# Zhongxu-Wang/ArtSpeech

Hardware: AMD Instinct MI355X
Metric: mel frames/sec (whole job; per-GPU = value / n_gpus), acoustic-model inference path, batch 32 x 200-frame utterances (higher is better)
Workload: dtype f32 (f16x3 split-operand MFMA, fp32 accumulate)

## Files before the change

artspeech_amd/csrc/conv_gemm.h:

```cpp
#pragma once
#include "artspeech_hip.h"
#include "common.h"
#include "conv_gemm_rule.h"
#include "operand_image.h"

#define OOB 0xFFFFFFFFu
#define OOBH 0x80000000u

int as_conv_gemm_h3_launch(const ConvGemmArgs* const* a, const int* S, int n, int choice, hipStream_t stream);
int as_split_f16x2_launch(const float* x, int ldx, int K, int N, int lrelu, float slope, uint16_t* xh, hipStream_t stream,
                          const int32_t* n_valid = nullptr);

static inline __host__ __device__ int as_kbx(int K) { return operand_image::kbx(K); }
static inline bool as_fills_tall_tile(int M) { return conv_gemm_rule::fills_tall_tile(M); }

static inline conv_gemm_rule::Shape as_conv_gemm_shape(const ConvGemmArgs& a)
{
    conv_gemm_rule::Shape s;
    s.M = a.M; s.N = a.N; s.K = a.K; s.Kp = a.Kp; s.T = a.T; s.K2 = a.K2;
    s.n_prod = a.n_prod ? a.n_prod : 3;
    s.n_groups = a.n_groups < 1 ? 1 : a.n_groups;
    s.group_cols = a.group_cols; s.ileave_u = a.ileave_u; s.act = a.act;
    s.x32 = a.X != nullptr; s.xh = a.Xh != nullptr; s.y32 = a.Y != nullptr; s.yh = a.Yh != nullptr; s.w32 = a.W != nullptr;
    s.res = a.res != nullptr; s.div_sqrt2 = a.div_sqrt2 != 0; s.transpose_out = a.transpose_out != 0;
    s.has_ws = a.ws != nullptr; s.ws_bytes = a.ws_bytes;
    return s;
}
size_t as_conv_gemm_shape_workspace(const conv_gemm_rule::Shape& s, bool set);

struct H3Taps {
    unsigned long long w0, w1, w2, w3;
    int wide;
};

static inline int h3_pack_taps(const ConvGemmArgs& a, H3Taps* out)
{
    H3Taps tp = {0, 0, 0, 0, 0};
    unsigned long long* w = &tp.w0;
    for (int t = 0; t < a.T; ++t)
        if (a.dh[t] < -7 || a.dh[t] > 7 || a.dw[t] < -7 || a.dw[t] > 7) tp.wide = 1;
    for (int t = 0; t < a.T; ++t) {
        if (tp.wide && (a.dh[t] != 0 || a.dw[t] < -127 || a.dw[t] > 127)) return AS_EINVAL;
        const int byte = tp.wide ? a.dw[t] + 128 : ((a.dh[t] + 8) << 4) | (a.dw[t] + 8);
        w[t >> 3] |= (unsigned long long)byte << ((t & 7) * 8);
    }
    *out = tp;
    return AS_OK;
}

#ifdef __HIPCC__
static __device__ __forceinline__ unsigned long long h3_tap_word(const H3Taps& tp, int t)
{
    const int s = t >> 3;
    const unsigned long long m0 = 0ull - (unsigned long long)(s == 0), m1 = 0ull - (unsigned long long)(s == 1),
                             m2 = 0ull - (unsigned long long)(s == 2), m3 = 0ull - (unsigned long long)(s == 3);
    return (tp.w0 & m0) | (tp.w1 & m1) | (tp.w2 & m2) | (tp.w3 & m3);
}

#endif

#ifdef __HIPCC__
typedef float f32x16 __attribute__((ext_vector_type(16)));
typedef float f32x4 __attribute__((ext_vector_type(4)));
typedef unsigned u32x2_t __attribute__((ext_vector_type(2)));
typedef _Float16 f16x8 __attribute__((ext_vector_type(8)));

static __device__ __forceinline__ f32x4 buf_load4(__amdgpu_buffer_rsrc_t r, unsigned voff, int soff)
{
    return __builtin_bit_cast(f32x4, __builtin_amdgcn_raw_buffer_load_b128(r, voff, soff, 0));
}
static __device__ __forceinline__ float buf_load1(__amdgpu_buffer_rsrc_t r, unsigned voff, int soff)
{
    return __builtin_bit_cast(float, __builtin_amdgcn_raw_buffer_load_b32(r, voff, soff, 0));
}
#define H3_MAXP 6
struct H3Prob {
    ConvGemmArgs a;
    H3Taps tp;
    int32_t wg0, wgs;
    int32_t tiles, S;
    int32_t col0, col1;
    int32_t pad0_, pad1_;
};
struct H3Multi {
    int32_t n, pad_;
    H3Prob p[H3_MAXP];
};

static __device__ __forceinline__ int logical_of(int local, int wgs)
{
    return (local & 7) * (wgs >> 3) + (local >> 3);
}

static __device__ __forceinline__ float div_sqrt2f(float x)
{
    const float c = 1.41421356237309504880f, rc = 0.70710678118654752440f;
    const float q = x * rc;
    return __builtin_fmaf(__builtin_fmaf(-q, c, x), rc, q);
}

template <int ACT>
static __device__ __forceinline__ float epi_act(float x, float slope)
{
    if (ACT == 1) x = x < 0.f ? 0.f : x;
    if (ACT == 2) x = x > 0.f ? x : slope * x;
    if (ACT == 3) x = tanhf(x);
    if (ACT == 4) x = fabsf(x);
    if (ACT == 5) x = x / (1.0f + expf(-x));
    return x;
}

static __device__ __forceinline__ void yh_store_tile(const ConvGemmArgs& a, __amdgpu_buffer_rsrc_t rsH, const float (&v)[16], int row0,
                                                     int col, int lk, int n_end)
{
    const unsigned NXy = operand_image::rows32(a.N);
    const int groups = 2 * as_kbx(a.M);
#pragma unroll
    for (int pr = 0; pr < 2; ++pr) {
        float t[8];
#pragma unroll
        for (int r = 0; r < 4; ++r) {
            float x0 = v[8 * pr + r], x1 = v[8 * pr + 4 + r];
            if (a.yh_lrelu) {
                x0 = x0 > 0.f ? x0 : a.in_slope * x0;
                x1 = x1 > 0.f ? x1 : a.in_slope * x1;
            }
            asm volatile("s_nop 1\n\tv_permlane32_swap_b32 %0, %1" : "+v"(x0), "+v"(x1));
            t[r] = x0;
            t[4 + r] = x1;
        }
        u32x4_t h, l;
        split2(t, h, l);
        const int g = (row0 >> 3) + 2 * pr + lk;
        const bool ok = col < n_end && g < groups;
        const unsigned off = ok ? operand_image::byte_off(operand_image::plane(g), col, NXy) : OOBH;
        __builtin_amdgcn_raw_buffer_store_b128(h, rsH, off, 0, 0);
        __builtin_amdgcn_raw_buffer_store_b128(l, rsH, off + 2u * NXy * 16u, 0, 0);
        if (col == 0 && g < groups) {
            const u32x4_t z = {0u, 0u, 0u, 0u};
            const unsigned offz = operand_image::byte_off(operand_image::plane(g), a.N, NXy);
            __builtin_amdgcn_raw_buffer_store_b128(z, rsH, offz, 0, 0);
            __builtin_amdgcn_raw_buffer_store_b128(z, rsH, offz + 2u * NXy * 16u, 0, 0);
        }
    }
}

template <int TM, int TN, bool DIV, int ACT, bool TR>
static __device__ __forceinline__ void epilogue_tiles(const ConvGemmArgs& a, const f32x16 (&acc)[TM][TN], int rbase, int cbase,
                                                      int l31, int lk, int grp, int n_end)
{
    const __amdgpu_buffer_rsrc_t rsB = __builtin_amdgcn_make_buffer_rsrc(
        const_cast<float*>(a.bias ? a.bias + (size_t)grp * a.M : nullptr), 0, a.bias ? a.M * 4 : 0, 0x00020000);
    const __amdgpu_buffer_rsrc_t rsR = __builtin_amdgcn_make_buffer_rsrc(
        const_cast<float*>(a.res), 0, a.res ? (int)((unsigned)a.M * a.ldr * 4u) : 0, 0x00020000);
    const __amdgpu_buffer_rsrc_t rsY = __builtin_amdgcn_make_buffer_rsrc(
        a.Y, 0, a.Y ? (int)((unsigned)(TR ? a.N : (a.ileave_u > 1 ? a.M / a.ileave_u : a.M)) * a.ldy * 4u) : 0, 0x00020000);
    const __amdgpu_buffer_rsrc_t rsH = __builtin_amdgcn_make_buffer_rsrc(
        a.Yh, 0, a.Yh ? (int)operand_image::desc_bytes(a.M, operand_image::rows32(a.N)) : 0, 0x00020000);
    const float sc = a.acc_scale;
    if (a.range_probe) {
        bool bad = false;
#pragma unroll
        for (int i = 0; i < TM; ++i)
#pragma unroll
            for (int jn = 0; jn < TN; ++jn)
#pragma unroll
                for (int e = 0; e < 16; ++e) bad |= !(fabsf(acc[i][jn][e]) <= 3.0e38f);
        if (bad) as_status_raise(a.status, AS_STATUS_F16_RANGE);
    }
    float bv[TM][16];
#pragma unroll
    for (int i = 0; i < TM; ++i)
#pragma unroll
        for (int e = 0; e < 16; ++e) bv[i][e] = 0.f;
    if (a.bias) {
#pragma unroll
        for (int i = 0; i < TM; ++i)
#pragma unroll
            for (int e = 0; e < 16; ++e)
                bv[i][e] = buf_load1(rsB, (unsigned)(rbase + i * 32 + (e & 3) + 8 * (e >> 2)) * 4u, 0);
    }
#pragma unroll
    for (int i = 0; i < TM; ++i) {
#pragma unroll
        for (int jn = 0; jn < TN; ++jn) {
            const int col = cbase + jn * 32 + l31;
            const int row0 = rbase + i * 32;
            const unsigned r_off = col < n_end ? (unsigned)(row0 * a.ldr + col) * 4u : OOBH;
            float v[16];
#pragma unroll
            for (int e = 0; e < 16; ++e) v[e] = 0.f;
            if (a.res) {
#pragma unroll
                for (int e = 0; e < 16; ++e) v[e] = buf_load1(rsR, r_off + (unsigned)(((e & 3) + 8 * (e >> 2)) * a.ldr * 4), 0);
            }
#pragma unroll
            for (int e = 0; e < 16; ++e) {
                float x = __builtin_fmaf(acc[i][jn][e], sc, bv[i][e]);
                x += v[e];
                if (DIV) x = div_sqrt2f(x);
                v[e] = epi_act<ACT>(x, a.act_slope);
            }
            if (TR) {
                const bool quad = (a.ldy & 3) == 0 && (reinterpret_cast<uintptr_t>(a.Y) & 15) == 0 && row0 + 28 <= a.M;
                const unsigned off = col < n_end ? (unsigned)(col * a.ldy + row0) * 4u : OOBH;
                if (quad) {
#pragma unroll
                    for (int q = 0; q < 4; ++q) {
                        const f32x4 t = {v[4 * q], v[4 * q + 1], v[4 * q + 2], v[4 * q + 3]};
                        __builtin_amdgcn_raw_buffer_store_b128(__builtin_bit_cast(u32x4_t, t), rsY, off + 32u * q, 0, 0);
                    }
                } else {
#pragma unroll
                    for (int e = 0; e < 16; ++e) {
                        const int dr = (e & 3) + 8 * (e >> 2);
                        __builtin_amdgcn_raw_buffer_store_b32(__builtin_bit_cast(unsigned, v[e]), rsY,
                                                              row0 + dr < a.M ? off + 4u * dr : OOBH, 0, 0);
                    }
                }
            } else {
                if (a.Y) {
                    unsigned off = col < n_end ? (unsigned)(row0 * a.ldy + col) * 4u : OOBH;
                    if (a.ileave_u > 1) {
                        const int Cc = a.M / a.ileave_u, r = (row0 - 4 * lk) / Cc;
                        off = (col < n_end && row0 - 4 * lk < a.M) ? (unsigned)((row0 - r * Cc) * a.ldy + a.ileave_u * col + r) * 4u : OOBH;
                    }
#pragma unroll
                    for (int e = 0; e < 16; ++e)
                        __builtin_amdgcn_raw_buffer_store_b32(__builtin_bit_cast(unsigned, v[e]), rsY,
                                                              off + (unsigned)(((e & 3) + 8 * (e >> 2)) * a.ldy * 4), 0, 0);
                }
                if (a.Yh) yh_store_tile(a, rsH, v, row0 - 4 * lk, col, lk, n_end);
            }
        }
    }
}

template <int TM, int TN, int AUX = 0>
static __device__ __forceinline__ void slab_store(const ConvGemmArgs& a, const f32x16 (&acc)[TM][TN], __amdgpu_buffer_rsrc_t rs,
                                                  int rbase, int cbase, int l31, int n_end)
{
#pragma unroll
    for (int i = 0; i < TM; ++i)
#pragma unroll
        for (int jn = 0; jn < TN; ++jn) {
            const int col = cbase + jn * 32 + l31;
            const unsigned v0 = col < n_end ? (unsigned)((rbase + i * 32) * a.N + col) * 4u : OOBH;
#pragma unroll
            for (int e = 0; e < 16; ++e) {
                float t = acc[i][jn][e];
                asm volatile("" : "+v"(t));
                __builtin_amdgcn_raw_buffer_store_b32(__builtin_bit_cast(unsigned, t), rs,
                                                      v0 + (unsigned)(((e & 3) + 8 * (e >> 2)) * a.N * 4), 0, AUX);
            }
        }
}

template <int TM, int TN>
static __device__ __forceinline__ void slab_store_tr(const ConvGemmArgs& a, const f32x16 (&acc)[TM][TN], __amdgpu_buffer_rsrc_t rs,
                                                     int rbase, int cbase, int l31, int n_end)
{
#pragma unroll
    for (int i = 0; i < TM; ++i)
#pragma unroll
        for (int jn = 0; jn < TN; ++jn) {
            const int col = cbase + jn * 32 + l31;
#pragma unroll
            for (int q = 0; q < 4; ++q) {
                const int row = rbase + i * 32 + 8 * q;
                float t0 = acc[i][jn][4 * q], t1 = acc[i][jn][4 * q + 1], t2 = acc[i][jn][4 * q + 2], t3 = acc[i][jn][4 * q + 3];
                asm volatile("" : "+v"(t0), "+v"(t1), "+v"(t2), "+v"(t3));
                const f32x4 t = {t0, t1, t2, t3};
                const unsigned off = (col < n_end && row < a.M) ? (unsigned)(col * a.M + row) * 4u : OOBH;
                __builtin_amdgcn_raw_buffer_store_b128(__builtin_bit_cast(u32x4_t, t), rs, off, 0, 0);
            }
        }
}

template <bool LEAN = false>
static __device__ __forceinline__ float as_reduce_value(const ConvGemmArgs& a, float x, float bias, float res)
{
    if (a.range_probe && !(fabsf(x) <= 3.0e38f)) as_status_raise(a.status, AS_STATUS_F16_RANGE);
    x = __fmul_rn(x, a.acc_scale);
    if (a.bias) x = __fadd_rn(x, bias);
    if (a.res) x = __fadd_rn(x, res);
    if (a.div_sqrt2) x = __fdiv_rn(x, 1.41421356237309504880f);
    if (a.act == 1) x = x < 0.f ? 0.f : x;
    else if (a.act == 2) x = x > 0.f ? x : __fmul_rn(a.act_slope, x);
    else if (!LEAN) {
        if (a.act == 3) x = tanhf(x);
        else if (a.act == 4) x = fabsf(x);
        else if (a.act == 5) x = x / (1.0f + expf(-x));
    }
    return x;
}

static __device__ __forceinline__ void as_reduce_epilogue(const ConvGemmArgs& a, int S, int j, int g)
{
    if (j > a.N || (j == a.N && !a.Yh)) return;
    const size_t total = (size_t)a.M * a.N;
    const float* slab = reinterpret_cast<const float*>(a.ws);
    const int grp = a.n_groups > 1 ? (j < a.N ? j : a.N - 1) / a.group_cols : 0;
    if (a.n_valid && j < a.N && j - (a.n_groups > 1 ? grp * a.group_cols : 0) >= *a.n_valid) return;
    float acc8[8] = {0.f, 0.f, 0.f, 0.f, 0.f, 0.f, 0.f, 0.f};
    {
        const int jc = j < a.N ? j : a.N - 1;
        size_t idx[8];
#pragma unroll
        for (int r = 0; r < 8; ++r) {
            const int row = 8 * g + r;
            idx[r] = (size_t)(row < a.M ? row : a.M - 1) * a.N + jc;
        }
        int s = 0;
        for (; s + 4 <= S; s += 4) {
            float t[4][8];
#pragma unroll
            for (int u = 0; u < 4; ++u)
#pragma unroll
                for (int r = 0; r < 8; ++r) t[u][r] = slab[(size_t)(s + u) * total + idx[r]];
#pragma unroll
            for (int u = 0; u < 4; ++u)
#pragma unroll
                for (int r = 0; r < 8; ++r) acc8[r] += t[u][r];
        }
        for (; s < S; ++s) {
            float t[8];
#pragma unroll
            for (int r = 0; r < 8; ++r) t[r] = slab[(size_t)s * total + idx[r]];
#pragma unroll
            for (int r = 0; r < 8; ++r) acc8[r] += t[r];
        }
    }
    float bias8[8], res8[8];
#pragma unroll
    for (int r = 0; r < 8; ++r) {
        const int row = 8 * g + r < a.M ? 8 * g + r : a.M - 1;
        bias8[r] = a.bias ? a.bias[(size_t)grp * a.M + row] : 0.f;
        res8[r] = a.res ? a.res[(size_t)row * a.ldr + (j < a.N ? j : a.N - 1)] : 0.f;
    }
    float v[8];
#pragma unroll
    for (int r = 0; r < 8; ++r) {
        const int row = 8 * g + r;
        float x = 0.f;
        if (row < a.M && j < a.N) {
            x = as_reduce_value(a, acc8[r], bias8[r], res8[r]);
            if (a.Y) {
                if (a.transpose_out) a.Y[(size_t)j * a.ldy + row] = x;
                else a.Y[(size_t)row * a.ldy + j] = x;
            }
        }
        v[r] = x;
    }
    if (a.Yh && g < 2 * as_kbx(a.M)) {
        if (a.yh_lrelu) {
#pragma unroll
            for (int r = 0; r < 8; ++r) v[r] = v[r] > 0.f ? v[r] : a.in_slope * v[r];
        }
        u32x4_t h, l;
        split2(v, h, l);
        const size_t NX = operand_image::rows(a.N);
        oi_store(reinterpret_cast<u32x4_t*>(a.Yh) + operand_image::row(g, 0, j, NX), 0, NX, h, l);
    }
}

template <int TM, int TN>
static __device__ __forceinline__ void epilogue_dispatch(const ConvGemmArgs& a, const f32x16 (&acc)[TM][TN], int rbase, int cbase,
                                                         int l31, int lk, int grp, int n_end)
{
    if (a.transpose_out) epilogue_tiles<TM, TN, false, 0, true>(a, acc, rbase, cbase, l31, lk, grp, n_end);
    else if (a.div_sqrt2 && a.act == 0) epilogue_tiles<TM, TN, true, 0, false>(a, acc, rbase, cbase, l31, lk, grp, n_end);
    else if (a.div_sqrt2 && a.act == 2) epilogue_tiles<TM, TN, true, 2, false>(a, acc, rbase, cbase, l31, lk, grp, n_end);
    else if (a.div_sqrt2) epilogue_tiles<TM, TN, true, 1, false>(a, acc, rbase, cbase, l31, lk, grp, n_end);
    else if (a.act == 0) epilogue_tiles<TM, TN, false, 0, false>(a, acc, rbase, cbase, l31, lk, grp, n_end);
    else if (a.act == 1) epilogue_tiles<TM, TN, false, 1, false>(a, acc, rbase, cbase, l31, lk, grp, n_end);
    else if (a.act == 3) epilogue_tiles<TM, TN, false, 3, false>(a, acc, rbase, cbase, l31, lk, grp, n_end);
    else if (a.act == 4) epilogue_tiles<TM, TN, false, 4, false>(a, acc, rbase, cbase, l31, lk, grp, n_end);
    else if (a.act == 5) epilogue_tiles<TM, TN, false, 5, false>(a, acc, rbase, cbase, l31, lk, grp, n_end);
    else epilogue_tiles<TM, TN, false, 2, false>(a, acc, rbase, cbase, l31, lk, grp, n_end);
}

template <int TM, int TN>
static __device__ __forceinline__ void epilogue(const ConvGemmArgs& a, const f32x16 (&acc)[TM][TN], int m0, int n0, int wm,
                                                int wn, int l31, int lk, int S, int slice, bool active, int grp, int n_end)
{
    if (!active) return;
    const int rbase = m0 + wm * 32 * TM + 4 * lk;
    const int cbase = n0 + wn * 32 * TN;
    if (S == 1) {
        epilogue_dispatch<TM, TN>(a, acc, rbase, cbase, l31, lk, grp, n_end);
        return;
    }
    const __amdgpu_buffer_rsrc_t rs = __builtin_amdgcn_make_buffer_rsrc(
        reinterpret_cast<float*>(a.ws) + (size_t)slice * a.M * a.N, 0, (int)((unsigned)a.M * a.N * 4u), 0x00020000);
    if (a.slab_tr) slab_store_tr<TM, TN>(a, acc, rs, rbase, cbase, l31, n_end);
    else slab_store<TM, TN>(a, acc, rs, rbase, cbase, l31, n_end);
}
#endif
```

artspeech_amd/csrc/conv_gemm_h3.hip:

```cpp
#include "conv_gemm.h"
#include <cstring>
#include <type_traits>

typedef __attribute__((address_space(3))) void lds_void;

template <int I, int N, typename F>
static __device__ __forceinline__ void h3_for(F&& f)
{
    if constexpr (I < N) {
        f(std::integral_constant<int, I>{});
        h3_for<I + 1, N>(f);
    }
}

template <int WM, int WN, int WK, int KT, int NS, int NP, int TM = 2>
struct H3Cfg {
    static constexpr int QP = NP == 1 ? 2 : 4;
    static constexpr int BM = 32 * TM * WM, BN = 64 * WN;
    static constexpr int KBS = WK * KT;
    static constexpr int A_BLK = QP * BM * 16, B_BLK = QP * BN * 16;
    static constexpr int A_ST = KBS * A_BLK;
    static constexpr int STAGE = KBS * (A_BLK + B_BLK);
    static constexpr int RED = (WK - 1) * WM * WN * 32 * TM * 64 * 4;
    static constexpr int LDS = NS * STAGE > RED ? NS * STAGE : RED;
    static constexpr int NT = 64 * WM * WN * WK;
    static constexpr int ACH = KBS * QP * BM / NT;
    static constexpr int BCH = KBS * QP * BN / NT;
    static constexpr int NMF = 2 * TM * NP;
    static constexpr int NFR = (TM + 2) * (NP == 1 ? 1 : 2);
};

static constexpr int H3_OCC = 1;
static __device__ __forceinline__ int h3_problem_of(const H3Multi& mm)
{
    int pi = 0;
#pragma unroll
    for (int i = 1; i < H3_MAXP; ++i) pi += (i < mm.n && (int)blockIdx.x >= mm.p[i].wg0) ? 1 : 0;
    return pi;
}

template <int WM, int WN, int WK, int KT, int NS, int NP, int TM = 2>
static __device__ __forceinline__ void h3_tile(const H3Prob& prob, unsigned char* smem)
{
    using C = H3Cfg<WM, WN, WK, KT, NS, NP, TM>;
    static_assert(NS >= 2 && NS <= 4, "stages");
    constexpr int BM = C::BM, BN = C::BN, ACH = C::ACH, BCH = C::BCH, NT = C::NT, QP = C::QP, KBS = C::KBS;
    static_assert(NT == 256 && ACH * NT == KBS * QP * BM && BCH * NT == KBS * QP * BN && ACH >= 1 && BCH >= 1, "tile shape");

    const int tid = threadIdx.x, lane = tid & 63;
    const int wave = __builtin_amdgcn_readfirstlane(tid >> 6);
    const int wk = wave / (WM * WN), wmn = wave % (WM * WN), wm = wmn % WM, wn = wmn / WM;
    const int l31 = lane & 31, lk = lane >> 5;
    const ConvGemmArgs& a = prob.a;
    const H3Taps& tp = prob.tp;
    const int S = prob.S;
    const int tiles_m = (a.M + BM - 1) / BM;
    int lt, slice, tile, m0, n0, grp = 0, n_end = prob.col1;
    if (a.n_valid && S == 1) {
        const int nv = __builtin_amdgcn_readfirstlane(*a.n_valid);
        const int G = a.n_groups > 1 ? a.n_groups : 1;
        const int span = G > 1 ? a.group_cols : prob.col1 - prob.col0;
        const int ctv = (min(max(nv, 1), span) + BN - 1) / BN;
        const int tiles_v = tiles_m * G * ctv, per = (tiles_v + 7) >> 3;
        const int local = (int)blockIdx.x - prob.wg0;
        if ((local >> 3) >= per) return;
        lt = (local & 7) * per + (local >> 3);
        if (lt >= tiles_v) return;
        slice = 0;
        tile = lt;
        m0 = (lt % tiles_m) * BM;
        const int q = lt / tiles_m, tn = q / G;
        grp = q - tn * G;
        const int base = G > 1 ? grp * a.group_cols : prob.col0;
        n0 = base + tn * BN;
        n_end = min(G > 1 ? min(a.N, (grp + 1) * a.group_cols) : prob.col1, base + nv);
    } else {
        lt = logical_of((int)blockIdx.x - prob.wg0, prob.wgs);
        if (lt >= prob.tiles * S) return;
        slice = lt / prob.tiles;
        tile = lt - slice * prob.tiles;
        m0 = (tile % tiles_m) * BM;
        n0 = prob.col0 + (tile / tiles_m) * BN;
        if (a.n_groups > 1) {
            const int tpg = (a.group_cols + BN - 1) / BN, tn = tile / tiles_m;
            grp = tn / tpg;
            n0 = grp * a.group_cols + (tn - grp * tpg) * BN;
            n_end = min(a.N, (grp + 1) * a.group_cols);
        }
        if (a.n_valid) {
            n_end = min(n_end, (a.n_groups > 1 ? grp * a.group_cols : 0) + __builtin_amdgcn_readfirstlane(*a.n_valid));
            if (n0 >= n_end && n0 > 0) return;
        }
    }
    const int KB = a.Kp >> 4, KBx = (KB + 3) & ~3;
    const int NX = (a.src_col ? a.N_in : a.N) + 1;

    const int KB2 = (a.K2 + 15) >> 4, KBx2 = (KB2 + 3) & ~3;
    const unsigned w_bytes = ((unsigned)a.T * KBx + KBx2) * 4u * a.M * 16u;
    const __amdgpu_buffer_rsrc_t rsW = __builtin_amdgcn_make_buffer_rsrc(
        const_cast<unsigned char*>(reinterpret_cast<const unsigned char*>(a.Wh) + (size_t)grp * w_bytes), 0, (int)w_bytes, 0x00020000);
    const __amdgpu_buffer_rsrc_t rsX = __builtin_amdgcn_make_buffer_rsrc(
        const_cast<uint16_t*>(a.Xh), 0, (int)operand_image::desc_bytes_kb(KBx, NX), 0x00020000);
    const __amdgpu_buffer_rsrc_t rsX2 = __builtin_amdgcn_make_buffer_rsrc(
        const_cast<uint16_t*>(KB2 ? a.Xh2 : a.Xh), 0, (int)operand_image::desc_bytes_kb(KBx2, NX), 0x00020000);

    (void)rsW;
    (void)rsX;
    (void)rsX2;
    unsigned a_voff[ACH];
#pragma unroll
    for (int i = 0; i < ACH; ++i) {
        const int c = tid + NT * i, kblk = c / (QP * BM), rem = c % (QP * BM), pk = rem / BM, row = rem % BM;
        a_voff[i] = (m0 + row) < a.M ? (unsigned)(((kblk * 4 + pk) * a.M + m0 + row) * 16) : OOB;
    }
    unsigned b_plane[BCH];
#pragma unroll
    for (int i = 0; i < BCH; ++i) {
        const int c = tid + NT * i, kblk = c / (QP * BN), pk = (c % (QP * BN)) / BN;
        b_plane[i] = (unsigned)((kblk * 4 + pk) * NX) * 16u;
    }
    const int j = n0 + tid % BN;
    unsigned tapmask = 0;
    int Wj = 0;
    if (j < n_end) {
        if (a.meta) {
            const unsigned long long md = a.meta[j];
            const int h = AS_META_h(md), w = AS_META_w(md);
            const int H = AS_META_H(md);
            Wj = AS_META_W(md);
            for (int t = 0; t < a.T; ++t) {
                const int byte = (int)(h3_tap_word(tp, t) >> ((t & 7) * 8)) & 0xff;
                const int dh = tp.wide ? 0 : (byte >> 4) - 8, dw = tp.wide ? byte - 128 : (byte & 15) - 8;
                if ((unsigned)(h + dh) < (unsigned)H && (unsigned)(w + dw) < (unsigned)Wj) tapmask |= 1u << t;
            }
        } else {
            tapmask = 0xffffffffu;
        }
    }
    const int jsrc = a.src_col ? (j < n_end ? a.src_col[j] : 0) : j;
    const int tA = tp.wide ? 16 : Wj, tC = jsrc + (tp.wide ? -128 : -8 * Wj - 8);

    const int it_per_tap = (KB + KBS - 1) / KBS;
    const int nit_all = a.T * it_per_tap + (KB2 + KBS - 1) / KBS;
    const int it_lo = (int)((long)nit_all * slice / S);
    const int n_it = (int)((long)nit_all * (slice + 1) / S) - it_lo;

    int s_t = min(it_lo / it_per_tap, a.T), s_kb = (it_lo - s_t * it_per_tap) * KBS;
    int kb_lim = s_t < a.T ? KB : KB2;
    __amdgpu_buffer_rsrc_t rsXc = s_t < a.T ? rsX : rsX2;
    const int a_step = KBS * 4 * a.M * 16, b_step = KBS * 4 * NX * 16;
    int a_soff = (s_t * KBx + s_kb) * 4 * a.M * 16, b_soff = s_kb * 4 * NX * 16;
    unsigned bv[BCH];
    auto set_tap = [&](int t) {
        int byte = (int)(h3_tap_word(tp, t) >> ((t & 7) * 8)) & 0xff;
        unsigned ok = 0u - ((tapmask >> (t & 31)) & 1u);
        if (t >= a.T) {
            byte = tp.wide ? 128 : 0x88;
            ok = 0u - (unsigned)(j < n_end);
        }
        const unsigned src = ((unsigned)((byte >> 4) * tA + (byte & 15) + tC) & ok) | ((unsigned)(NX - 1) & ~ok);
#pragma unroll
        for (int i = 0; i < BCH; ++i) bv[i] = b_plane[i] + src * 16u;
    };
    set_tap(s_t);
    auto advance = [&]() {
        s_kb += KBS;
        a_soff += a_step;
        b_soff += b_step;
        if (s_kb >= kb_lim) {
            if (s_t + 1 < a.T || (s_t + 1 == a.T && KB2 > 0)) {
                s_t += 1;
                s_kb = 0;
                a_soff = s_t * KBx * 4 * a.M * 16;
                b_soff = 0;
                if (s_t == a.T) {
                    kb_lim = KB2;
                    rsXc = rsX2;
                }
                set_tap(s_t);
            } else {
                s_kb -= KBS;
                a_soff -= a_step;
                b_soff -= b_step;
            }
        }
    };
    auto dma_a = [&](auto i_, int stage) {
#if __HIP_DEVICE_COMPILE__
        constexpr int i = decltype(i_)::value;
        __builtin_amdgcn_raw_ptr_buffer_load_lds(rsW, (lds_void*)(smem + stage * C::STAGE + wave * 1024 + i * (NT * 16)), 16, a_voff[i],
                                                 a_soff, 0, 0);
#endif
    };
    auto dma_b = [&](auto i_, int stage) {
#if __HIP_DEVICE_COMPILE__
        constexpr int i = decltype(i_)::value;
        __builtin_amdgcn_raw_ptr_buffer_load_lds(rsXc, (lds_void*)(smem + stage * C::STAGE + C::A_ST + wave * 1024 + i * (NT * 16)), 16, bv[i],
                                                 b_soff, 0, 0);
#endif
    };
    (void)bv;
    (void)a_soff;
    (void)b_soff;
    (void)rsXc;
    f16x8 fa[2][TM][2], fb[2][2][2];
    const int a_frag = (wk * KT * QP + lk) * BM * 16 + (wm * 32 * TM + l31) * 16;
    const int b_frag = C::A_ST + (wk * KT * QP + lk) * BN * 16 + (wn * 64 + l31) * 16;
    auto read_frag = [&](auto q_, auto set_, auto s_, int stage) {
        constexpr int q = decltype(q_)::value, set = decltype(set_)::value, s = decltype(s_)::value;
        constexpr int sec = q < TM ? 0 : (q < TM + 2 ? 1 : (q < 2 * TM + 2 ? 2 : 3));
        constexpr int i = sec == 0 ? q : (sec == 1 ? q - TM : (sec == 2 ? q - TM - 2 : q - 2 * TM - 2));
        constexpr int ab = sec == 0 || sec == 2 ? 0 : 1;
        constexpr int p = NP == 1 ? 0 : (sec == 0 || sec == 3 ? 0 : 1);
        const unsigned char* st = smem + stage * C::STAGE;
        if constexpr (ab == 0) fa[set][i][p] = *reinterpret_cast<const f16x8*>(st + a_frag + (s * QP + p * 2) * BM * 16 + i * 32 * 16);
        else fb[set][i][p] = *reinterpret_cast<const f16x8*>(st + b_frag + (s * QP + p * 2) * BN * 16 + i * 32 * 16);
    };
    f32x16 acc[TM][2];
#pragma unroll
    for (int i = 0; i < TM; ++i)
#pragma unroll
        for (int jn = 0; jn < 2; ++jn)
#pragma unroll
            for (int e = 0; e < 16; ++e) acc[i][jn][e] = 0.f;

    using I0 = std::integral_constant<int, 0>;
    constexpr int L = KT == 1 ? NS : NS - 1;
    static_assert(L >= 2, "KT > 1 needs three stages");
    for (int st = 0; st < L; ++st) {
        h3_for<0, ACH>([&](auto i_) { dma_a(i_, st); });
        h3_for<0, BCH>([&](auto i_) { dma_b(i_, st); });
        advance();
    }
    __syncthreads();
    h3_for<0, C::NFR>([&](auto q_) { read_frag(q_, I0{}, I0{}, 0); });
    __syncthreads();

    constexpr int NMI = KT * C::NMF;
    constexpr int M_ADV = ACH + BCH, NMS = M_ADV + 1;
    constexpr int SLOT0 = 0;
    auto stage_micro = [&](auto m_, auto p_) {
        constexpr int Mi = decltype(m_)::value, P = (decltype(p_)::value + L) % NS;
        if constexpr (Mi < ACH) dma_a(std::integral_constant<int, Mi>{}, P);
        else if constexpr (Mi < M_ADV) dma_b(std::integral_constant<int, Mi - ACH>{}, P);
        else advance();
    };
    auto slot_of_stage = [](int m) constexpr { return SLOT0 + (m * (NMI - SLOT0)) / NMS; };
    auto slot_of_frag = [](int s, int q) constexpr {
        return s * C::NMF + (q * (C::NMF - 2)) / C::NFR + (C::NMF > 4 ? 1 : 0);
    };
    auto step = [&](auto n_, auto s_, auto p_, auto f_) {
        constexpr int Nn = decltype(n_)::value, Ss = decltype(s_)::value, P = decltype(p_)::value, F = decltype(f_)::value;
        constexpr int grp_ = Nn / (2 * TM), i = (Nn % (2 * TM)) / 2, jn = Nn % 2;
        constexpr int PA = NP == 1 ? 0 : (grp_ == 1 ? 1 : 0);
        constexpr int PB = NP == 1 ? 0 : (grp_ == 0 ? 1 : 0);
        acc[i][jn] = __builtin_amdgcn_mfma_f32_32x32x16_f16(fa[F][i][PA], fb[F][jn][PB], acc[i][jn], 0, 0, 0);
        constexpr int slot = Ss * C::NMF + Nn;
        h3_for<0, NMS>([&](auto m_) {
            if constexpr (slot_of_stage(decltype(m_)::value) == slot) stage_micro(m_, p_);
        });
        h3_for<0, C::NFR>([&](auto q_) {
            if constexpr (slot_of_frag(Ss, decltype(q_)::value) == slot) {
                if constexpr (Ss + 1 < KT) read_frag(q_, std::integral_constant<int, F ^ 1>{}, std::integral_constant<int, Ss + 1>{}, P);
                else read_frag(q_, std::integral_constant<int, F ^ 1>{}, I0{}, (P + 1) % NS);
            }
        });
        __builtin_amdgcn_sched_barrier(0);
    };
    constexpr int PEND = (L - 2) * (ACH + BCH);
#define H3_ITER(U)                                                                                                \
    {                                                                                                             \
        h3_for<0, KT>([&](auto s_) {                                                                              \
            h3_for<0, C::NMF>([&](auto n_) {                                                                      \
                step(n_, s_, std::integral_constant<int, (U) % NS>{},                                             \
                     std::integral_constant<int, ((U) * KT + decltype(s_)::value) % 2>{});                        \
            });                                                                                                   \
        });                                                                                                       \
        asm volatile("s_waitcnt vmcnt(%0) lgkmcnt(0)\n\ts_barrier" ::"n"(PEND) : "memory");                     \
    }
    constexpr int PERIOD = (KT % 2 == 0) ? NS : (NS % 2 == 0 ? NS : 2 * NS);
    int it = 0;
    for (; it + PERIOD <= n_it; it += PERIOD) {
        h3_for<0, PERIOD>([&](auto u_) { H3_ITER(decltype(u_)::value) });
    }
    h3_for<0, PERIOD - 1>([&](auto u_) {
        if (it + decltype(u_)::value < n_it) H3_ITER(decltype(u_)::value)
    });
#undef H3_ITER
    asm volatile("s_waitcnt vmcnt(0)\n\ts_barrier" ::: "memory");

    if (WK > 1) {
        f32x4* red = reinterpret_cast<f32x4*>(smem);
        if (wk > 0) {
#pragma unroll
            for (int i = 0; i < TM; ++i)
#pragma unroll
                for (int jn = 0; jn < 2; ++jn)
#pragma unroll
                    for (int e4 = 0; e4 < 4; ++e4) {
                        f32x4 v = {acc[i][jn][4 * e4], acc[i][jn][4 * e4 + 1], acc[i][jn][4 * e4 + 2], acc[i][jn][4 * e4 + 3]};
                        red[((((wk - 1) * (WM * WN) + wmn) * 2 * TM + i * 2 + jn) * 4 + e4) * 64 + lane] = v;
                    }
        }
        __syncthreads();
        if (wk == 0)
#pragma unroll
            for (int s = 1; s < WK; ++s)
#pragma unroll
                for (int i = 0; i < TM; ++i)
#pragma unroll
                    for (int jn = 0; jn < 2; ++jn)
#pragma unroll
                        for (int e4 = 0; e4 < 4; ++e4) {
                            const f32x4 v = red[((((s - 1) * (WM * WN) + wmn) * 2 * TM + i * 2 + jn) * 4 + e4) * 64 + lane];
#pragma unroll
                            for (int c = 0; c < 4; ++c) acc[i][jn][4 * e4 + c] += v[c];
                        }
    }
    epilogue<TM, 2>(a, acc, m0, n0, wm, wn, l31, lk, S, slice, wk == 0, grp, n_end);
}

template <int WM, int WN, int WK, int KT, int NS, int NP, int TM = 2>
__global__ void __launch_bounds__(64 * WM * WN * WK, H3_OCC)
conv_gemm_h3_kernel(const H3Multi mm)
{
    extern __shared__ __attribute__((aligned(16))) unsigned char smem[];
    h3_tile<WM, WN, WK, KT, NS, NP, TM>(mm.p[h3_problem_of(mm)], smem);
}

template <int WM, int WN, int WK, int KT, int NS, int NP, int TM = 2>
static int launch_h3(const ConvGemmArgs* const* a, const int* S, int n, hipStream_t stream)
{
    using C = H3Cfg<WM, WN, WK, KT, NS, NP, TM>;
    AS_LDS_OPT_IN((&conv_gemm_h3_kernel<WM, WN, WK, KT, NS, NP, TM>), C::LDS);
    H3Multi mm;
    memset(&mm, 0, sizeof(mm));
    mm.n = n;
    int wg = 0;
    for (int i = 0; i < n; ++i) {
        H3Prob& p = mm.p[i];
        p.a = *a[i];
        if (h3_pack_taps(p.a, &p.tp) != AS_OK) return AS_EINVAL;
        const int tiles_n = p.a.n_groups > 1 ? p.a.n_groups * as_cdiv(p.a.group_cols, C::BN) : as_cdiv(p.a.N, C::BN);
        p.tiles = as_cdiv(p.a.M, C::BM) * tiles_n;
        p.col0 = 0;
        p.col1 = p.a.N;
        p.S = S[i];
        p.wg0 = wg;
        p.wgs = (p.tiles * p.S + 7) & ~7;
        wg += p.wgs;
    }
    hipLaunchKernelGGL((conv_gemm_h3_kernel<WM, WN, WK, KT, NS, NP, TM>), dim3(wg), dim3(C::NT), C::LDS, stream, mm);
    AS_CHECK_LAUNCH();
    return AS_OK;
}

template <int WM, int WN, int WK>
static int launch_h3_tile(const ConvGemmArgs* const* a, const int* S, int n, hipStream_t stream)
{
    if (a[0]->n_prod == 1) return launch_h3<WM, WN, WK, 1, 3, 1>(a, S, n, stream);
    return launch_h3<WM, WN, WK, 1, 3, 3>(a, S, n, stream);
}

int as_conv_gemm_h3_launch(const ConvGemmArgs* const* a, const int* S, int n, int choice, hipStream_t stream)
{
    if (n < 1 || n > H3_MAXP) return AS_EINVAL;
    for (int i = 0; i < n; ++i) {
        if (a[i]->n_prod != a[0]->n_prod || S[i] < 1) return AS_EINVAL;
        if (operand_image::bytes(a[i]->K, a[i]->src_col ? a[i]->N_in : a[i]->N) >= ((size_t)1 << 31)) return AS_EINVAL;
    }
    switch (choice) {
    case 2:
        if (a[0]->n_prod == 1) return AS_EINVAL;
        return launch_h3<1, 2, 2, 1, 2, 3, 1>(a, S, n, stream);
    case 22: return launch_h3_tile<2, 2, 1>(a, S, n, stream);
    case 21: return launch_h3_tile<2, 1, 2>(a, S, n, stream);
    case 12: return launch_h3_tile<1, 2, 2>(a, S, n, stream);
    case 14:
        if (a[0]->n_prod == 1) return launch_h3_tile<1, 2, 2>(a, S, n, stream);
        return launch_h3<1, 4, 1, 1, 3, 3>(a, S, n, stream);
    case 11: return launch_h3_tile<1, 1, 4>(a, S, n, stream);
    default: return AS_EINVAL;
    }
}

__global__ void __launch_bounds__(256)
split_f16x2_kernel(const float* __restrict__ x, int ldx, int K, int N, const int* __restrict__ n_valid, int lrelu, float slope,
                   u32x4_t* __restrict__ xh)
{
    const int wcol = (blockIdx.x * 256 + (threadIdx.x & ~63)) * 4;
    const int col = wcol + (threadIdx.x & 63);
    const int g = blockIdx.y;
    if (wcol > N) return;
    const int nv = n_valid ? min(max(*n_valid, 0), N) : N;
    if (wcol >= nv && wcol + 255 < N) return;
    const __amdgpu_buffer_rsrc_t rs = __builtin_amdgcn_make_buffer_rsrc(const_cast<float*>(x), 0, (int)(((unsigned)(K - 1) * ldx + N) * 4u), 0x00020000);
    float v[8][4];
#pragma unroll
    for (int r = 0; r < 8; ++r) {
        const int k = g * 8 + r;
#pragma unroll
        for (int c = 0; c < 4; ++c) v[r][c] = buf_load1(rs, (k < K && col + 64 * c < nv) ? (unsigned)(k * ldx + col + 64 * c) * 4u : OOB, 0);
    }
    const size_t NX = operand_image::rows(N);
    const size_t base = operand_image::row(g, 0, col, NX);
#pragma unroll
    for (int c = 0; c < 4; ++c) {
        if (col + 64 * c > N) break;
        if (col + 64 * c >= nv && col + 64 * c < N) continue;
        float t[8];
#pragma unroll
        for (int r = 0; r < 8; ++r) {
            float e = v[r][c];
            if (lrelu) e = e > 0.f ? e : slope * e;
            t[r] = e;
        }
        oi_store(xh, base + 64 * c, NX, t);
    }
}

extern "C" size_t as_split_f16x2_bytes(int K, int N)
{
    return conv_gemm_rule::split_f16x2_bytes(K, N);
}

int as_split_f16x2_launch(const float* x, int ldx, int K, int N, int lrelu, float slope, uint16_t* xh, hipStream_t stream,
                          const int32_t* n_valid)
{
    if ((double)K * ldx * 4.0 >= 2147483648.0) return AS_EINVAL;
    hipLaunchKernelGGL(split_f16x2_kernel, dim3(as_cdiv(N + 1, 1024), 2 * as_kbx(K)), dim3(256), 0, stream, x, ldx, K, N, n_valid, lrelu, slope,
                       reinterpret_cast<u32x4_t*>(xh));
    AS_CHECK_LAUNCH();
    return AS_OK;
}

extern "C" int as_split_f16x2_f32(const float* x, int ldx, int K, int N, int in_act, float in_slope, uint16_t* xh, as_stream_t stream)
{
    return as_split_f16x2_cap_f32(x, ldx, K, N, nullptr, in_act, in_slope, xh, stream);
}

extern "C" int as_split_f16x2_cap_f32(const float* x, int ldx, int K, int N, const int32_t* n_valid, int in_act, float in_slope, uint16_t* xh,
                                      as_stream_t stream)
{
    if (!x || !xh || K <= 0 || N < 0 || ldx < N || (in_act != 0 && in_act != 2) || !(fabsf(in_slope) <= 3.0e38f)) return AS_EINVAL;
    if ((reinterpret_cast<uintptr_t>(xh) & 15) != 0) return AS_EINVAL;
    if (N == 0) return AS_OK;
    AsProfScope prof__(AS_CLS_OTHER, 0, 8.0 * K * (double)N, (hipStream_t)stream);
    return as_split_f16x2_launch(x, ldx, K, N, in_act == 2, in_slope, xh, (hipStream_t)stream, n_valid);
}

extern "C" size_t as_prep_weight_f16x2_sc_bytes(int G, int Cout, int Cin, int T, int Cin2)
{
    if (G <= 0 || Cout <= 0 || Cin <= 0 || T <= 0 || Cin2 < 0) return 0;
    return (size_t)G * ((size_t)T * as_kbx(Cin) + (Cin2 ? as_kbx(Cin2) : 0)) * 4 * (size_t)Cout * 16;
}
extern "C" size_t as_prep_weight_f16x2_bytes(int G, int Cout, int Cin, int T) { return as_prep_weight_f16x2_sc_bytes(G, Cout, Cin, T, 0); }

extern "C" int as_prep_weight_f16x2_sc_host(const float* w, const float* w2, int G, int Cout, int Cin, int T, int Cin2, uint16_t* wh,
                                            float* scale_out)
{
    if (!w || !wh || !scale_out || G <= 0 || Cout <= 0 || Cin <= 0 || T <= 0 || Cin2 < 0 || ((Cin2 > 0) != (w2 != nullptr))) return AS_EINVAL;
    const size_t n = (size_t)G * Cout * Cin * T, n2 = (size_t)G * Cout * Cin2;
    float mx = 0.f;
    for (size_t i = 0; i < n + n2; ++i) {
        const float x = i < n ? w[i] : w2[i - n];
        const float v = x < 0 ? -x : x;
        if (!(v <= 3.0e38f)) return AS_EINVAL;
        mx = v > mx ? v : mx;
    }
    int e = 0;
    float scale = 1.0f;
    if (mx > 0.f) {
        frexpf(mx, &e);
        scale = ldexpf(1.0f, 14 - e);
    }
    const int KBx = as_kbx(Cin), KBx2 = Cin2 ? as_kbx(Cin2) : 0;
// ... 367 lines not shown
```

Measured before the change: 1.795 million.

## Peel pipelined GEMM tail, relax prologue waits, and prefetch bias via bpermute

Restructures the h3 conv-GEMM main loop so the last lookahead iterations are peeled into tail iterations that issue no further LDS-DMA stages or next-tile fragment reads and skip unneeded barriers. The prologue now waits only on the oldest tiles with a partial vmcnt instead of full __syncthreads. The per-element bias loads in the epilogue become a single per-lane load issued before the tail, redistributed with ds_bpermute. Launch-bounds occupancy is raised from 1 to 2 or 4 depending on TM, which may constrain register allocation. A host-side schedule checker is added to validate the ordering.

```diff
diff --git a/artspeech_amd/csrc/conv_gemm.h b/artspeech_amd/csrc/conv_gemm.h
--- a/artspeech_amd/csrc/conv_gemm.h
+++ b/artspeech_amd/csrc/conv_gemm.h
@@ -145,12 +145,19 @@
     }
 }
 
-template <int TM, int TN, bool DIV, int ACT, bool TR>
-static __device__ __forceinline__ void epilogue_tiles(const ConvGemmArgs& a, const f32x16 (&acc)[TM][TN], int rbase, int cbase,
-                                                      int l31, int lk, int grp, int n_end)
+static __device__ __forceinline__ float epilogue_bias(const ConvGemmArgs& a, int row0, int lane, int grp, bool wanted)
 {
     const __amdgpu_buffer_rsrc_t rsB = __builtin_amdgcn_make_buffer_rsrc(
         const_cast<float*>(a.bias ? a.bias + (size_t)grp * a.M : nullptr), 0, a.bias ? a.M * 4 : 0, 0x00020000);
+    float b = 0.f;
+    if (a.bias && wanted) b = buf_load1(rsB, (unsigned)(row0 + lane) * 4u, 0);
+    return b;
+}
+
+template <int TM, int TN, bool DIV, int ACT, bool TR>
+static __device__ __forceinline__ void epilogue_tiles(const ConvGemmArgs& a, const f32x16 (&acc)[TM][TN], float bias,
+                                                      int rbase, int cbase, int l31, int lk, int grp, int n_end)
+{
     const __amdgpu_buffer_rsrc_t rsR = __builtin_amdgcn_make_buffer_rsrc(
         const_cast<float*>(a.res), 0, a.res ? (int)((unsigned)a.M * a.ldr * 4u) : 0, 0x00020000);
     const __amdgpu_buffer_rsrc_t rsY = __builtin_amdgcn_make_buffer_rsrc(
@@ -158,6 +165,13 @@
     const __amdgpu_buffer_rsrc_t rsH = __builtin_amdgcn_make_buffer_rsrc(
         a.Yh, 0, a.Yh ? (int)operand_image::desc_bytes(a.M, operand_image::rows32(a.N)) : 0, 0x00020000);
     const float sc = a.acc_scale;
+    float bv[TM][16];
+#pragma unroll
+    for (int i = 0; i < TM; ++i)
+#pragma unroll
+        for (int e = 0; e < 16; ++e)
+            bv[i][e] = __builtin_bit_cast(float, __builtin_amdgcn_ds_bpermute((i * 32 + (e & 3) + 8 * (e >> 2) + 4 * lk) << 2,
+                                                                              __builtin_bit_cast(int, bias)));
     if (a.range_probe) {
         bool bad = false;
 #pragma unroll
@@ -167,18 +181,6 @@
 #pragma unroll
                 for (int e = 0; e < 16; ++e) bad |= !(fabsf(acc[i][jn][e]) <= 3.0e38f);
         if (bad) as_status_raise(a.status, AS_STATUS_F16_RANGE);
-    }
-    float bv[TM][16];
-#pragma unroll
-    for (int i = 0; i < TM; ++i)
-#pragma unroll
-        for (int e = 0; e < 16; ++e) bv[i][e] = 0.f;
-    if (a.bias) {
-#pragma unroll
-        for (int i = 0; i < TM; ++i)
-#pragma unroll
-            for (int e = 0; e < 16; ++e)
-                bv[i][e] = buf_load1(rsB, (unsigned)(rbase + i * 32 + (e & 3) + 8 * (e >> 2)) * 4u, 0);
     }
 #pragma unroll
     for (int i = 0; i < TM; ++i) {
@@ -365,30 +367,30 @@
 }
 
 template <int TM, int TN>
-static __device__ __forceinline__ void epilogue_dispatch(const ConvGemmArgs& a, const f32x16 (&acc)[TM][TN], int rbase, int cbase,
+static __device__ __forceinline__ void epilogue_dispatch(const ConvGemmArgs& a, const f32x16 (&acc)[TM][TN], float bias, int rbase, int cbase,
                                                          int l31, int lk, int grp, int n_end)
 {
-    if (a.transpose_out) epilogue_tiles<TM, TN, false, 0, true>(a, acc, rbase, cbase, l31, lk, grp, n_end);
-    else if (a.div_sqrt2 && a.act == 0) epilogue_tiles<TM, TN, true, 0, false>(a, acc, rbase, cbase, l31, lk, grp, n_end);
-    else if (a.div_sqrt2 && a.act == 2) epilogue_tiles<TM, TN, true, 2, false>(a, acc, rbase, cbase, l31, lk, grp, n_end);
-    else if (a.div_sqrt2) epilogue_tiles<TM, TN, true, 1, false>(a, acc, rbase, cbase, l31, lk, grp, n_end);
-    else if (a.act == 0) epilogue_tiles<TM, TN, false, 0, false>(a, acc, rbase, cbase, l31, lk, grp, n_end);
-    else if (a.act == 1) epilogue_tiles<TM, TN, false, 1, false>(a, acc, rbase, cbase, l31, lk, grp, n_end);
-    else if (a.act == 3) epilogue_tiles<TM, TN, false, 3, false>(a, acc, rbase, cbase, l31, lk, grp, n_end);
-    else if (a.act == 4) epilogue_tiles<TM, TN, false, 4, false>(a, acc, rbase, cbase, l31, lk, grp, n_end);
-    else if (a.act == 5) epilogue_tiles<TM, TN, false, 5, false>(a, acc, rbase, cbase, l31, lk, grp, n_end);
-    else epilogue_tiles<TM, TN, false, 2, false>(a, acc, rbase, cbase, l31, lk, grp, n_end);
+    if (a.transpose_out) epilogue_tiles<TM, TN, false, 0, true>(a, acc, bias, rbase, cbase, l31, lk, grp, n_end);
+    else if (a.div_sqrt2 && a.act == 0) epilogue_tiles<TM, TN, true, 0, false>(a, acc, bias, rbase, cbase, l31, lk, grp, n_end);
+    else if (a.div_sqrt2 && a.act == 2) epilogue_tiles<TM, TN, true, 2, false>(a, acc, bias, rbase, cbase, l31, lk, grp, n_end);
+    else if (a.div_sqrt2) epilogue_tiles<TM, TN, true, 1, false>(a, acc, bias, rbase, cbase, l31, lk, grp, n_end);
+    else if (a.act == 0) epilogue_tiles<TM, TN, false, 0, false>(a, acc, bias, rbase, cbase, l31, lk, grp, n_end);
+    else if (a.act == 1) epilogue_tiles<TM, TN, false, 1, false>(a, acc, bias, rbase, cbase, l31, lk, grp, n_end);
+    else if (a.act == 3) epilogue_tiles<TM, TN, false, 3, false>(a, acc, bias, rbase, cbase, l31, lk, grp, n_end);
+    else if (a.act == 4) epilogue_tiles<TM, TN, false, 4, false>(a, acc, bias, rbase, cbase, l31, lk, grp, n_end);
+    else if (a.act == 5) epilogue_tiles<TM, TN, false, 5, false>(a, acc, bias, rbase, cbase, l31, lk, grp, n_end);
+    else epilogue_tiles<TM, TN, false, 2, false>(a, acc, bias, rbase, cbase, l31, lk, grp, n_end);
 }
 
 template <int TM, int TN>
-static __device__ __forceinline__ void epilogue(const ConvGemmArgs& a, const f32x16 (&acc)[TM][TN], int m0, int n0, int wm,
-                                                int wn, int l31, int lk, int S, int slice, bool active, int grp, int n_end)
+static __device__ __forceinline__ void epilogue(const ConvGemmArgs& a, const f32x16 (&acc)[TM][TN], float bias, int m0, int n0,
+                                                int wm, int wn, int l31, int lk, int S, int slice, bool active, int grp, int n_end)
 {
     if (!active) return;
     const int rbase = m0 + wm * 32 * TM + 4 * lk;
     const int cbase = n0 + wn * 32 * TN;
     if (S == 1) {
-        epilogue_dispatch<TM, TN>(a, acc, rbase, cbase, l31, lk, grp, n_end);
+        epilogue_dispatch<TM, TN>(a, acc, bias, rbase, cbase, l31, lk, grp, n_end);
         return;
     }
     const __amdgpu_buffer_rsrc_t rs = __builtin_amdgcn_make_buffer_rsrc(
diff --git a/artspeech_amd/csrc/conv_gemm_h3.hip b/artspeech_amd/csrc/conv_gemm_h3.hip
--- a/artspeech_amd/csrc/conv_gemm_h3.hip
+++ b/artspeech_amd/csrc/conv_gemm_h3.hip
@@ -1,4 +1,5 @@
 #include "conv_gemm.h"
+#include "conv_gemm_loop.h"
 #include <cstring>
 #include <type_traits>
 
@@ -30,7 +31,7 @@
     static constexpr int NFR = (TM + 2) * (NP == 1 ? 1 : 2);
 };
 
-static constexpr int H3_OCC = 1;
+static constexpr int h3_occ(int TM) { return TM == 1 ? 4 : 2; }
 static __device__ __forceinline__ int h3_problem_of(const H3Multi& mm)
 {
     int pi = 0;
@@ -225,16 +226,20 @@
             for (int e = 0; e < 16; ++e) acc[i][jn][e] = 0.f;
 
     using I0 = std::integral_constant<int, 0>;
-    constexpr int L = KT == 1 ? NS : NS - 1;
-    static_assert(L >= 2, "KT > 1 needs three stages");
+    namespace gl = conv_gemm_loop;
+    static_assert(gl::valid(NS, KT), "KT > 1 needs three stages");
+    constexpr int L = gl::lookahead(NS, KT);
+    constexpr int PEND = gl::pend_tiles(NS, KT) * (ACH + BCH);
+    constexpr int PRO = gl::prologue_tiles(NS, KT) * (ACH + BCH);
+    static_assert(PRO < 64, "vmcnt is six bits");
     for (int st = 0; st < L; ++st) {
         h3_for<0, ACH>([&](auto i_) { dma_a(i_, st); });
         h3_for<0, BCH>([&](auto i_) { dma_b(i_, st); });
         advance();
     }
-    __syncthreads();
+    asm volatile("s_waitcnt vmcnt(%0)\n\ts_barrier" ::"n"(PRO) : "memory");
     h3_for<0, C::NFR>([&](auto q_) { read_frag(q_, I0{}, I0{}, 0); });
-    __syncthreads();
+    asm volatile("s_waitcnt vmcnt(%0) lgkmcnt(0)\n\ts_barrier" ::"n"(PEND) : "memory");
 
     constexpr int NMI = KT * C::NMF;
     constexpr int M_ADV = ACH + BCH, NMS = M_ADV + 1;
@@ -249,45 +254,70 @@
     auto slot_of_frag = [](int s, int q) constexpr {
         return s * C::NMF + (q * (C::NMF - 2)) / C::NFR + (C::NMF > 4 ? 1 : 0);
     };
-    auto step = [&](auto n_, auto s_, auto p_, auto f_) {
+    auto step = [&](auto n_, auto s_, auto p_, auto f_, auto stg_, auto nxt_) {
         constexpr int Nn = decltype(n_)::value, Ss = decltype(s_)::value, P = decltype(p_)::value, F = decltype(f_)::value;
         constexpr int grp_ = Nn / (2 * TM), i = (Nn % (2 * TM)) / 2, jn = Nn % 2;
         constexpr int PA = NP == 1 ? 0 : (grp_ == 1 ? 1 : 0);
         constexpr int PB = NP == 1 ? 0 : (grp_ == 0 ? 1 : 0);
         acc[i][jn] = __builtin_amdgcn_mfma_f32_32x32x16_f16(fa[F][i][PA], fb[F][jn][PB], acc[i][jn], 0, 0, 0);
         constexpr int slot = Ss * C::NMF + Nn;
-        h3_for<0, NMS>([&](auto m_) {
-            if constexpr (slot_of_stage(decltype(m_)::value) == slot) stage_micro(m_, p_);
-        });
+        if constexpr (decltype(stg_)::value)
+            h3_for<0, NMS>([&](auto m_) {
+                if constexpr (slot_of_stage(decltype(m_)::value) == slot) stage_micro(m_, p_);
+            });
         h3_for<0, C::NFR>([&](auto q_) {
             if constexpr (slot_of_frag(Ss, decltype(q_)::value) == slot) {
                 if constexpr (Ss + 1 < KT) read_frag(q_, std::integral_constant<int, F ^ 1>{}, std::integral_constant<int, Ss + 1>{}, P);
-                else read_frag(q_, std::integral_constant<int, F ^ 1>{}, I0{}, (P + 1) % NS);
+                else if constexpr (decltype(nxt_)::value) read_frag(q_, std::integral_constant<int, F ^ 1>{}, I0{}, (P + 1) % NS);
             }
         });
         __builtin_amdgcn_sched_barrier(0);
     };
-    constexpr int PEND = (L - 2) * (ACH + BCH);
-#define H3_ITER(U)                                                                                                \
-    {                                                                                                             \
-        h3_for<0, KT>([&](auto s_) {                                                                              \
-            h3_for<0, C::NMF>([&](auto n_) {                                                                      \
-                step(n_, s_, std::integral_constant<int, (U) % NS>{},                                             \
-                     std::integral_constant<int, ((U) * KT + decltype(s_)::value) % 2>{});                        \
-            });                                                                                                   \
-        });                                                                                                       \
-        asm volatile("s_waitcnt vmcnt(%0) lgkmcnt(0)\n\ts_barrier" ::"n"(PEND) : "memory");                     \
-    }
-    constexpr int PERIOD = (KT % 2 == 0) ? NS : (NS % 2 == 0 ? NS : 2 * NS);
+    constexpr int END_STAGED = 0, END_DRAIN = 1, END_READS = 2, END_NONE = 3;
+    auto iter = [&](auto u_, auto stg_, auto nxt_, auto end_) {
+        constexpr int U = decltype(u_)::value, END = decltype(end_)::value;
+        h3_for<0, KT>([&](auto s_) {
+            h3_for<0, C::NMF>([&](auto n_) {
+                step(n_, s_, std::integral_constant<int, U % NS>{}, std::integral_constant<int, (U * KT + decltype(s_)::value) % 2>{}, stg_, nxt_);
+            });
+        });
+        if constexpr (END == END_STAGED) asm volatile("s_waitcnt vmcnt(%0) lgkmcnt(0)\n\ts_barrier" ::"n"(PEND) : "memory");
+        else if constexpr (END == END_DRAIN) asm volatile("s_waitcnt vmcnt(0) lgkmcnt(0)\n\ts_barrier" ::: "memory");
+        else if constexpr (END == END_READS) asm volatile("s_waitcnt lgkmcnt(0)" ::: "memory");
+    };
+    using Yes = std::true_type;
+    using No = std::false_type;
+    auto staged_iter = [&](auto u_) { iter(u_, Yes{}, Yes{}, std::integral_constant<int, END_STAGED>{}); };
+    auto tail_iter = [&](auto u_, auto j_, auto count_) {
+        constexpr int j = decltype(j_)::value, count = decltype(count_)::value;
+        constexpr bool nxt = gl::tail_reads_next(j, count);
+        iter(u_, No{}, std::integral_constant<bool, nxt>{}, std::integral_constant<int, gl::tail_drains(j) ? END_DRAIN : (nxt ? END_READS : END_NONE)>{});
+    };
+    constexpr int PERIOD = gl::period(NS, KT);
+    const int n_main = gl::n_staged(n_it, NS, KT);
     int it = 0;
-    for (; it + PERIOD <= n_it; it += PERIOD) {
-        h3_for<0, PERIOD>([&](auto u_) { H3_ITER(decltype(u_)::value) });
+    for (; it + PERIOD <= n_main; it += PERIOD) {
+        h3_for<0, PERIOD>([&](auto u_) { staged_iter(u_); });
     }
     h3_for<0, PERIOD - 1>([&](auto u_) {
-        if (it + decltype(u_)::value < n_it) H3_ITER(decltype(u_)::value)
+        if (it + decltype(u_)::value < n_main) staged_iter(u_);
     });
-#undef H3_ITER
-    asm volatile("s_waitcnt vmcnt(0)\n\ts_barrier" ::: "memory");
+    const float bias = epilogue_bias(a, m0 + wm * 32 * TM, lane, grp, S == 1 && wk == 0);
+    if (n_it >= L) {
+        const int ph = n_main % PERIOD;
+        h3_for<0, PERIOD>([&](auto p_) {
+            if (ph == decltype(p_)::value)
+                h3_for<0, L>([&](auto j_) {
+                    tail_iter(std::integral_constant<int, (decltype(p_)::value + decltype(j_)::value) % PERIOD>{}, j_, std::integral_constant<int, L>{});
+                });
+        });
+    } else {
+        h3_for<1, L>([&](auto c_) {
+            if (n_it == decltype(c_)::value) h3_for<0, decltype(c_)::value>([&](auto j_) { tail_iter(j_, j_, c_); });
+        });
+        if (n_it <= 0) asm volatile("s_waitcnt vmcnt(0)" ::: "memory");
+    }
+    if (WK > 1) asm volatile("s_barrier" ::: "memory");
 
     if (WK > 1) {
         f32x4* red = reinterpret_cast<f32x4*>(smem);
@@ -317,11 +347,11 @@
                             for (int c = 0; c < 4; ++c) acc[i][jn][4 * e4 + c] += v[c];
                         }
     }
-    epilogue<TM, 2>(a, acc, m0, n0, wm, wn, l31, lk, S, slice, wk == 0, grp, n_end);
+    epilogue<TM, 2>(a, acc, bias, m0, n0, wm, wn, l31, lk, S, slice, wk == 0, grp, n_end);
 }
 
 template <int WM, int WN, int WK, int KT, int NS, int NP, int TM = 2>
-__global__ void __launch_bounds__(64 * WM * WN * WK, H3_OCC)
+__global__ void __launch_bounds__(64 * WM * WN * WK, h3_occ(TM))
 conv_gemm_h3_kernel(const H3Multi mm)
 {
     extern __shared__ __attribute__((aligned(16))) unsigned char smem[];
diff --git a/artspeech_amd/csrc/conv_gemm_loop.h b/artspeech_amd/csrc/conv_gemm_loop.h
--- /dev/null
+++ b/artspeech_amd/csrc/conv_gemm_loop.h
@@ -0,0 +1,135 @@
+#pragma once
+#include <string>
+#include <vector>
+
+namespace conv_gemm_loop {
+
+constexpr int lookahead(int NS, int KT) { return KT == 1 ? NS : NS - 1; }
+constexpr int period(int NS, int KT) { return (KT % 2 == 0) ? NS : (NS % 2 == 0 ? NS : 2 * NS); }
+constexpr int pend_tiles(int NS, int KT) { return lookahead(NS, KT) - 2; }
+constexpr int prologue_tiles(int NS, int KT) { return lookahead(NS, KT) - 1; }
+constexpr bool valid(int NS, int KT) { return NS >= 2 && NS <= 4 && KT >= 1 && lookahead(NS, KT) >= 2; }
+
+constexpr int n_staged(int n_it, int NS, int KT) { return n_it > lookahead(NS, KT) ? n_it - lookahead(NS, KT) : 0; }
+constexpr int n_tail(int n_it, int NS, int KT) { return n_it < lookahead(NS, KT) ? (n_it > 0 ? n_it : 0) : lookahead(NS, KT); }
+
+constexpr bool tail_drains(int j) { return j == 0; }
+constexpr bool tail_reads_next(int j, int count) { return j + 1 < count; }
+
+struct Iter {
+    int phase;
+    int stage;
+    int set;
+    int stage_tile;
+    bool reads_next;
+    int wait_tiles;
+    bool barrier;
+};
+
+constexpr Iter iteration(int n_it, int NS, int KT, int it)
+{
+    const int L = lookahead(NS, KT), ns = n_staged(n_it, NS, KT);
+    Iter r{it % period(NS, KT), it % NS, (it * KT) % 2, -1, true, -1, false};
+    if (it < ns) {
+        r.stage_tile = it + L;
+        r.wait_tiles = pend_tiles(NS, KT);
+        r.barrier = true;
+    } else {
+        const int j = it - ns;
+        r.reads_next = tail_reads_next(j, n_tail(n_it, NS, KT));
+        r.wait_tiles = tail_drains(j) ? 0 : -1;
+        r.barrier = tail_drains(j);
+    }
+    return r;
+}
+
+struct Op {
+    enum Kind { STAGE, READ, WAIT_VM, WAIT_LGKM, BARRIER } kind;
+    int tile;
+    int slot;
+    int step;
+};
+
+inline std::vector<Op> schedule(int n_it, int NS, int KT)
+{
+    std::vector<Op> ops;
+    const int L = lookahead(NS, KT);
+    for (int t = 0; t < L; ++t) ops.push_back({Op::STAGE, t, t % NS, 0});
+    ops.push_back({Op::WAIT_VM, prologue_tiles(NS, KT), 0, 0});
+    ops.push_back({Op::BARRIER, 0, 0, 0});
+    ops.push_back({Op::READ, 0, 0, 0});
+    ops.push_back({Op::WAIT_VM, pend_tiles(NS, KT), 0, 0});
+    ops.push_back({Op::WAIT_LGKM, 0, 0, 0});
+    ops.push_back({Op::BARRIER, 0, 0, 0});
+    for (int it = 0; it < n_it; ++it) {
+        const Iter i = iteration(n_it, NS, KT, it);
+        if (i.stage_tile >= 0) ops.push_back({Op::STAGE, i.stage_tile, i.stage_tile % NS, 0});
+        for (int s = 1; s < KT; ++s) ops.push_back({Op::READ, it, i.stage, s});
+        if (i.reads_next) ops.push_back({Op::READ, it + 1, (it + 1) % NS, 0});
+        if (i.wait_tiles >= 0) ops.push_back({Op::WAIT_VM, i.wait_tiles, 0, 0});
+        if (i.wait_tiles >= 0 || i.reads_next || KT > 1) ops.push_back({Op::WAIT_LGKM, 0, 0, 0});
+        if (i.barrier) ops.push_back({Op::BARRIER, 0, 0, 0});
+    }
+    if (n_it <= 0) ops.push_back({Op::WAIT_VM, 0, 0, 0});
+    return ops;
+}
+
+inline std::string check(const std::vector<Op>& ops, int n_it, int NS, int KT)
+{
+    enum { NONE, ISSUED, LANDED, PUBLISHED };
+    struct Slot { int tile = -1, state = NONE; bool read = false, written = false; };
+    std::vector<Slot> slot(NS);
+    std::vector<int> flight;
+    bool lgkm = false;
+    int next_read = 0;
+    auto at = [](size_t i) { return " (operation " + std::to_string(i) + ")"; };
+    for (size_t i = 0; i < ops.size(); ++i) {
+        const Op& o = ops[i];
+        switch (o.kind) {
+        case Op::STAGE: {
+            if (o.slot < 0 || o.slot >= NS) return "stage out of range" + at(i);
+            Slot& s = slot[o.slot];
+            if (s.read) return "a stage is restaged while a wave may still read it" + at(i);
+            if (s.state == ISSUED) return "a stage is restaged while its tile is in flight" + at(i);
+            s.tile = o.tile;
+            s.state = ISSUED;
+            s.written = true;
+            flight.push_back(o.slot);
+            break;
+        }
+        case Op::READ: {
+            if (o.slot < 0 || o.slot >= NS) return "stage out of range" + at(i);
+            Slot& s = slot[o.slot];
+            if (s.tile != o.tile) return "a read finds another tile in its stage" + at(i);
+            if (s.state != PUBLISHED) return "a read of a tile that has not landed and been published" + at(i);
+            if (s.written) return "a read of a stage written since the last barrier" + at(i);
+            if (o.tile * KT + o.step != next_read) return "fragments read out of order" + at(i);
+            ++next_read;
+            s.read = true;
+            lgkm = true;
+            break;
+        }
+        case Op::WAIT_VM:
+            while ((int)flight.size() > o.tile) {
+                slot[flight.front()].state = LANDED;
+                flight.erase(flight.begin());
+            }
+            break;
+        case Op::WAIT_LGKM: lgkm = false; break;
+        case Op::BARRIER:
+            if (lgkm) return "a barrier with fragment reads not waited for" + at(i);
+            for (Slot& s : slot) {
+                if (s.state == LANDED) s.state = PUBLISHED;
+                s.read = s.written = false;
+            }
+            break;
+        }
+    }
+    if (!flight.empty()) return "LDS-DMAs in flight at exit";
+    if (lgkm) return "fragment reads not waited for at exit";
+    const int want = n_it > 0 ? n_it * KT : 1;
+    if (next_read != want) return "the share's fragments were not all read: " + std::to_string(next_read) + " of " + std::to_string(want);
+    return "";
+}
+
+}
```

Result: no change. 1.798 million (median of 2 runs) (+0.2%).
